# daniel05155/Reinforcement-Learning-in-Music-Generation

Measured on AMD Instinct MI355X. Metric: CW-tokens/sec pretrain fwd+bwd @T=1024, higher is better.
Workload: dtype bf16; 1 GPU; agent_pretrain step (fwd+bwd+clip+Adam), repo dims 512/12/8/2048, synthetic CW tokens (B=512/GPU, T=1024, 7 fields -> 6); per_gpu_batch=512, global_batch=512, seq_len=1024, parallelism=dp1, params=38982227, gemm_table=True

## Files before the change

reinforcement-learning-in-music-generation_amd/csrc/cwlt_common.h:

```cpp
#pragma once
#include <hip/hip_runtime.h>
#include <stdint.h>

#define CWLT_OK 0
#define CWLT_ERR_ARG 1001
#define CWLT_ERR_DTYPE 1002

#define CWLT_F32 0
#define CWLT_BF16 1

typedef float f32x16 __attribute__((ext_vector_type(16)));
typedef float f32x4 __attribute__((ext_vector_type(4)));
typedef uint16_t bf16_t;

namespace cwlt {

constexpr int WAVE = 64;

typedef unsigned int u32x4_t __attribute__((ext_vector_type(4)));
__device__ __forceinline__ __amdgpu_buffer_rsrc_t make_rsrc(const void* base, uint32_t bytes) {
    return __builtin_amdgcn_make_buffer_rsrc(const_cast<void*>(base), (short)0, (int)bytes, 0x00020000);
}
__device__ __forceinline__ uint4 buf_load16(__amdgpu_buffer_rsrc_t r, uint32_t byte_off) {
    const u32x4_t v = __builtin_amdgcn_raw_buffer_load_b128(r, (int)byte_off, 0, 0);
    return make_uint4(v[0], v[1], v[2], v[3]);
}

#define CWLT_U4Z make_uint4(0u, 0u, 0u, 0u)

__device__ __forceinline__ float bf16_to_f32(bf16_t x) { return __uint_as_float(((uint32_t)x) << 16); }

typedef __bf16 hwbf16x2 __attribute__((ext_vector_type(2)));
__device__ __forceinline__ bf16_t f32_to_bf16(float f) { return __builtin_bit_cast(bf16_t, (__bf16)f); }
__device__ __forceinline__ uint32_t f32x2_to_bf16x2(float lo, float hi) {
    hwbf16x2 v;
    v[0] = (__bf16)lo;
    v[1] = (__bf16)hi;
    return __builtin_bit_cast(uint32_t, v);
}

__device__ __forceinline__ float4 load4(const float* p) { return *reinterpret_cast<const float4*>(p); }
__device__ __forceinline__ float4 load4(const bf16_t* p) {
    uint2 r = *reinterpret_cast<const uint2*>(p);
    float4 f;
    f.x = __uint_as_float(r.x << 16);
    f.y = __uint_as_float(r.x & 0xffff0000u);
    f.z = __uint_as_float(r.y << 16);
    f.w = __uint_as_float(r.y & 0xffff0000u);
    return f;
}
__device__ __forceinline__ void store4(float* p, float4 f) { *reinterpret_cast<float4*>(p) = f; }
__device__ __forceinline__ void store4(bf16_t* p, float4 f) {
    uint2 r;
    r.x = f32x2_to_bf16x2(f.x, f.y);
    r.y = f32x2_to_bf16x2(f.z, f.w);
    *reinterpret_cast<uint2*>(p) = r;
}
__device__ __forceinline__ float load1(const float* p) { return *p; }
__device__ __forceinline__ float load1(const bf16_t* p) { return bf16_to_f32(*p); }
__device__ __forceinline__ void store1(float* p, float f) { *p = f; }
__device__ __forceinline__ void store1(bf16_t* p, float f) { *p = f32_to_bf16(f); }

__device__ __forceinline__ void load8(const float* p, float (&x)[8]) {
    float4 a = load4(p), b = load4(p + 4);
    x[0] = a.x; x[1] = a.y; x[2] = a.z; x[3] = a.w; x[4] = b.x; x[5] = b.y; x[6] = b.z; x[7] = b.w;
}
__device__ __forceinline__ void load8(const bf16_t* p, float (&x)[8]) {
    uint4 r = *reinterpret_cast<const uint4*>(p);
    x[0] = __uint_as_float(r.x << 16); x[1] = __uint_as_float(r.x & 0xffff0000u);
    x[2] = __uint_as_float(r.y << 16); x[3] = __uint_as_float(r.y & 0xffff0000u);
    x[4] = __uint_as_float(r.z << 16); x[5] = __uint_as_float(r.z & 0xffff0000u);
    x[6] = __uint_as_float(r.w << 16); x[7] = __uint_as_float(r.w & 0xffff0000u);
}
__device__ __forceinline__ void store8(float* p, const float (&x)[8]) {
    store4(p, make_float4(x[0], x[1], x[2], x[3]));
    store4(p + 4, make_float4(x[4], x[5], x[6], x[7]));
}
__device__ __forceinline__ void store8(bf16_t* p, const float (&x)[8]) {
    uint4 r;
    r.x = f32x2_to_bf16x2(x[0], x[1]);
    r.y = f32x2_to_bf16x2(x[2], x[3]);
    r.z = f32x2_to_bf16x2(x[4], x[5]);
    r.w = f32x2_to_bf16x2(x[6], x[7]);
    *reinterpret_cast<uint4*>(p) = r;
}

template <typename T> struct VecIO;
template <> struct VecIO<float> {
    static constexpr int N = 4;
    static __device__ __forceinline__ void load(const float* p, float (&x)[4]) {
        const float4 a = load4(p);
        x[0] = a.x; x[1] = a.y; x[2] = a.z; x[3] = a.w;
    }
    static __device__ __forceinline__ void store(float* p, const float (&x)[4]) {
        store4(p, make_float4(x[0], x[1], x[2], x[3]));
    }
};
template <> struct VecIO<bf16_t> {
    static constexpr int N = 8;
    static __device__ __forceinline__ void load(const bf16_t* p, float (&x)[8]) { load8(p, x); }
    static __device__ __forceinline__ void store(bf16_t* p, const float (&x)[8]) { store8(p, x); }
};
template <int N>
__device__ __forceinline__ void loadf(const float* p, float (&x)[N]) {
#pragma unroll
    for (int i = 0; i < N; i += 4) {
        const float4 a = load4(p + i);
        x[i] = a.x; x[i + 1] = a.y; x[i + 2] = a.z; x[i + 3] = a.w;
    }
}

template <int CTRL>
__device__ __forceinline__ float dpp_move(float v) {
    return __builtin_bit_cast(float, __builtin_amdgcn_update_dpp(0, __builtin_bit_cast(int, v), CTRL, 0xf, 0xf, false));
}
__device__ __forceinline__ float lane_value(float v, int lane) {
    return __builtin_bit_cast(float, __builtin_amdgcn_readlane(__builtin_bit_cast(int, v), lane));
}
__device__ __forceinline__ float wave_sum(float v) {
    v += dpp_move<0xB1>(v);
    v += dpp_move<0x4E>(v);
    v += dpp_move<0x141>(v);
    v += dpp_move<0x140>(v);
    return (lane_value(v, 0) + lane_value(v, 16)) + (lane_value(v, 32) + lane_value(v, 48));
}
__device__ __forceinline__ float wave_max(float v) {
    v = fmaxf(v, dpp_move<0xB1>(v));
    v = fmaxf(v, dpp_move<0x4E>(v));
    v = fmaxf(v, dpp_move<0x141>(v));
    v = fmaxf(v, dpp_move<0x140>(v));
    return fmaxf(fmaxf(lane_value(v, 0), lane_value(v, 16)), fmaxf(lane_value(v, 32), lane_value(v, 48)));
}

__device__ __forceinline__ uint32_t hash32(uint32_t x) {
    x ^= x >> 16; x *= 0x7feb352du; x ^= x >> 15; x *= 0x846ca68bu; x ^= x >> 16;
    return x;
}
__device__ __forceinline__ uint32_t rng_pair(uint64_t seed, uint64_t pair_idx) {
    const uint32_t lo = (uint32_t)pair_idx, hi = (uint32_t)(pair_idx >> 32);
    const uint32_t key = (uint32_t)seed ^ ((uint32_t)(seed >> 32) * 0x9e3779b9u) ^ (hi * 0x85ebca6bu);
    return hash32(lo * 0x9e3779b1u ^ key);
}
template <int N>
__device__ __forceinline__ uint32_t dropout_mask(uint64_t seed, uint64_t off, uint32_t thresh16) {
    uint32_t m = 0;
#pragma unroll
    for (int j = 0; j < N; j += 2) {
        const uint32_t r = rng_pair(seed, (off >> 1) + (j >> 1));
        m |= ((r & 0xffffu) >= thresh16 ? 1u : 0u) << j;
        m |= ((r >> 16) >= thresh16 ? 1u : 0u) << (j + 1);
    }
    return m;
}
__device__ __forceinline__ bool dropout_keep(uint64_t seed, uint64_t idx, uint32_t thresh16) {
    const uint32_t r = rng_pair(seed, idx >> 1);
    return ((idx & 1) ? (r >> 16) : (r & 0xffffu)) >= thresh16;
}
__device__ __forceinline__ uint32_t keep_lanes16(uint32_t r, uint32_t thresh2) {
    uint32_t m;
    const uint32_t one = 0x00010001u;
    asm("v_pk_sub_u16 %0, %1, %2 clamp\n\t"
        "v_pk_min_u16 %0, %0, %3\n\t"
        "v_pk_sub_u16 %0, %0, %3"
        : "=&v"(m)
        : "s"(thresh2), "v"(r), "s"(one));
    return m;
}

static inline uint32_t drop_thresh(float p) {
    if (p <= 0.f) return 0u;
    long t = (long)((double)p * 65536.0 + 0.5);
    if (t < 1) t = 1;
    if (t > 65535) t = 65535;
    return (uint32_t)t;
}
static inline float drop_scale(float p) {
    const uint32_t t = drop_thresh(p);
    return t ? (float)(65536.0 / (65536.0 - (double)t)) : 1.0f;
}
int launch_colsum_finalize(const float* part, float* out, int nblocks, long stride, int ncols, float scale,
                           int accumulate, hipStream_t st);
int launch_colsum_finalize_multi(const float* part, float* out, long out_stride, int nq, int nblocks, long stride,
                                 int ncols, hipStream_t st);


int launch_gemm_ffn_big(int gelu, const void* a, const void* w, const float* bias, void* g, void* c, float* part,
                        int64_t M, int N, int K, int64_t lda, int64_t ldw, uint32_t thresh, float keep_scale,
                        uint64_t seed, const uint64_t* seed_base, hipStream_t st);
long gemm_ffn_big_tiles(long M);

int scan_segments(int N, int H, int L);
long scan_seg_floats(int N, int H, int P, int backward);
long scan_final_state_floats(int N, int H);
int launch_cla_fwd_bf16(const void* q, const void* k, const void* v, void* out, float* zinv, int N, int H, int L,
                        long ldq, long ldk, long ldv, long ldo, float eps, int P, float* ws, float* fin,
                        hipStream_t st);
int launch_cla_bwd_sweep_bf16(const void* q, const void* k, const void* v, const void* out, const float* zinv,
                              const void* dout, const float* fin, void* dq, void* dk, void* dv, float* csum_q,
                              float* csum_k, float* csum_v, int N, int H, int L, long ldq, long ldk, long ldv, long ldo,
                              long lddo, long lddq, long lddk, long lddv, hipStream_t st);
int launch_cla_bwd_dq_bf16(const void* q, const void* k, const void* v, const void* out, const float* zinv,
                           const void* dout, const float* dden, void* dq, float* csum, int N, int H, int L, long ldq,
                           long ldk, long ldv, long ldo, long lddo, long lddq, int P, float* ws, hipStream_t st);
int launch_cla_bwd_dkdv_bf16(const void* q, const void* k, const void* v, const void* out, const float* zinv,
                             const void* dout, void* dk, void* dv, float* csum_k, float* csum_v, float* dden_out,
                             int N, int H, int L, long ldq, long ldk, long ldv, long ldo, long lddo, long lddk,
                             long lddv, int P, float* ws, hipStream_t st);

}
```

reinforcement-learning-in-music-generation_amd/csrc/gemm_ln.hip:

```cpp
#include "cwlt_common.h"
#include "cwlt_lds_dma.h"
#include <stdlib.h>

namespace cwlt {
namespace gl {

constexpr int TMR = 128, TNC = 512, BK = 32;
constexpr int NSTAGE = 3;
constexpr int STG = (TMR + TNC) * BK * 2;
constexpr int LDE = TNC + 8;
constexpr int LDS_BYTES = TMR * LDE * 2 > NSTAGE * STG ? TMR * LDE * 2 : NSTAGE * STG;

typedef __bf16 bf16x4 __attribute__((ext_vector_type(4)));

__global__ __launch_bounds__(1024) void gemm_ln_kernel(
    const bf16_t* __restrict__ A, const bf16_t* __restrict__ W, const float* __restrict__ bias,
    const bf16_t* __restrict__ X, const float* __restrict__ gamma, const float* __restrict__ beta,
    bf16_t* __restrict__ S, bf16_t* __restrict__ Y, float* __restrict__ mean, float* __restrict__ rstd, long M, int K,
    long lda, long ldw, float eps, uint32_t thresh, float keep_scale, uint64_t seed,
    const uint64_t* __restrict__ seed_base) {
    extern __shared__ __attribute__((aligned(16))) char lds[];

    const int tid = threadIdx.x, lane = tid & 63;
    const int w = __builtin_amdgcn_readfirstlane(tid >> 6);
    const int wm = w >> 3, wn = w & 7;
    const int l31 = lane & 31, hf = lane >> 5;
    const long m0 = (long)blockIdx.x * TMR;
    const long mrows = min((long)TMR, M - m0);

    const uint64_t abase = (uint64_t)(A + m0 * lda), wbase = (uint64_t)W;
    u32x4_t ars, wrs;
    ars[0] = __builtin_amdgcn_readfirstlane((uint32_t)abase);
    ars[1] = __builtin_amdgcn_readfirstlane((uint32_t)(abase >> 32));
    ars[2] = __builtin_amdgcn_readfirstlane((uint32_t)(((mrows - 1) * lda + K) * 2));
    ars[3] = 0x00020000u;
    wrs[0] = __builtin_amdgcn_readfirstlane((uint32_t)wbase);
    wrs[1] = __builtin_amdgcn_readfirstlane((uint32_t)(wbase >> 32));
    wrs[2] = __builtin_amdgcn_readfirstlane((uint32_t)(((long)(TNC - 1) * ldw + K) * 2));
    wrs[3] = 0x00020000u;
    const int dchunk = (lane & 3) ^ ((lane >> 4) & 3);
    const uint32_t a_voff = ((uint32_t)(16 * (w & 7) + (lane >> 2)) * (uint32_t)lda + dchunk * 8) * 2;
    const uint32_t w_voff = ((uint32_t)(32 * w + (lane >> 2)) * (uint32_t)ldw + dchunk * 8) * 2;
    const uint32_t w_16 = (uint32_t)(16 * ldw * 2);
    const uint32_t lds_a = (uint32_t)(uintptr_t)(lds_void*)lds + (w & 7) * 1024;
    const uint32_t lds_w = (uint32_t)(uintptr_t)(lds_void*)lds + TMR * 64 + w * 2048;
#define GL_DMA_W(stage, step)                                                                                     \
    {                                                                                                             \
        unsigned keep;                                                                                            \
        const uint32_t lw = lds_w + (uint32_t)(stage) * STG;                                                      \
        const uint32_t sk_ = (uint32_t)(step) * (BK * 2), sk2 = sk_ + w_16;                                       \
        asm volatile("s_mov_b32 %0, m0\n\ts_mov_b32 m0, %2\n\ts_nop 4\n\t"                                     \
                     "buffer_load_dwordx4 %1, %3, %4 offen lds\n\t"                                               \
                     "s_add_u32 m0, %2, 0x400\n\ts_nop 0\n\t"                                                    \
                     "buffer_load_dwordx4 %1, %3, %5 offen lds\n\t"                                               \
                     "s_mov_b32 m0, %0"                                                                           \
                     : "=&s"(keep)                                                                                \
                     : "v"(w_voff), "s"(lw), "s"(wrs), "s"(sk_), "s"(sk2)                                         \
                     : "memory", "scc");                                                                          \
    }
#define GL_DMA_A(stage, step) lds_dma_piece(a_voff, ars, lds_a + (uint32_t)(stage) * STG, (uint32_t)(step) * (BK * 2))
#define GL_DMA(stage, step)        \
    {                              \
        if (w < 8) GL_DMA_A(stage, step); \
        GL_DMA_W(stage, step);     \
    }
    const int swz = (l31 >> 2) & 3;
    const int of0 = l31 * 64 + ((hf ^ swz) << 4), of1 = l31 * 64 + (((2 + hf) ^ swz) << 4);
    const int oa = (64 * wm) * 64, ow = TMR * 64 + (64 * wn) * 64;
#define GL_FRAG(p) __builtin_bit_cast(bf16x8, *reinterpret_cast<const uint4*>(p))
#define GL_READ(F, stage, ofh)                                            \
    {                                                                     \
        const char* sb = lds + (stage) * STG;                             \
        F[0] = GL_FRAG(sb + ow + (ofh));                                  \
        F[1] = GL_FRAG(sb + ow + 2048 + (ofh));                           \
        F[2] = GL_FRAG(sb + oa + (ofh));                                  \
        F[3] = GL_FRAG(sb + oa + 2048 + (ofh));                           \
    }
#define GL_MFMA(F)                                                                          \
    {                                                                                       \
        acc[0][0] = __builtin_amdgcn_mfma_f32_32x32x16_bf16(F[0], F[2], acc[0][0], 0, 0, 0); \
        acc[0][1] = __builtin_amdgcn_mfma_f32_32x32x16_bf16(F[1], F[2], acc[0][1], 0, 0, 0); \
        acc[1][0] = __builtin_amdgcn_mfma_f32_32x32x16_bf16(F[0], F[3], acc[1][0], 0, 0, 0); \
        acc[1][1] = __builtin_amdgcn_mfma_f32_32x32x16_bf16(F[1], F[3], acc[1][1], 0, 0, 0); \
    }

    f32x16 acc[2][2];
#pragma unroll
    for (int i = 0; i < 2; ++i)
#pragma unroll
        for (int j = 0; j < 2; ++j)
#pragma unroll
            for (int r = 0; r < 16; ++r) acc[i][j][r] = 0.f;

    const int nstep = K / BK;
    bf16x8 F0[4], F1[4];
    GL_DMA(0, 0);
    GL_DMA(1, 1);
    if (nstep > 2) GL_DMA(2, 2);
    if (nstep > 2) {
        if (w < 8)
            asm volatile("s_waitcnt vmcnt(6)" ::: "memory");
        else
            asm volatile("s_waitcnt vmcnt(4)" ::: "memory");
    } else {
        if (w < 8)
            asm volatile("s_waitcnt vmcnt(3)" ::: "memory");
        else
            asm volatile("s_waitcnt vmcnt(2)" ::: "memory");
    }
    __builtin_amdgcn_s_barrier();
    GL_READ(F0, 0, of0);
    int st = 0;
    for (int s = 0; s < nstep; ++s) {
        const int st1 = st == NSTAGE - 1 ? 0 : st + 1;
        GL_READ(F1, st, of1);
        __builtin_amdgcn_sched_barrier(0);
        GL_MFMA(F0);
        __builtin_amdgcn_sched_barrier(0);
        if (s + 1 < nstep) {
            if (s + 2 < nstep) {
                if (w < 8)
                    asm volatile("s_waitcnt vmcnt(3) lgkmcnt(0)" ::: "memory");
                else
                    asm volatile("s_waitcnt vmcnt(2) lgkmcnt(0)" ::: "memory");
            } else {
                asm volatile("s_waitcnt vmcnt(0) lgkmcnt(0)" ::: "memory");
            }
            __builtin_amdgcn_s_barrier();
            __builtin_amdgcn_sched_barrier(0);
            if (s + 3 < nstep) GL_DMA(st, s + 3);
            GL_READ(F0, st1, of0);
            __builtin_amdgcn_sched_barrier(0);
        }
        GL_MFMA(F1);
        __builtin_amdgcn_sched_barrier(0);
        st = st1;
    }
#undef GL_DMA
#undef GL_DMA_A
#undef GL_DMA_W
#undef GL_FRAG
#undef GL_READ
#undef GL_MFMA

    __syncthreads();
    bf16_t* et = reinterpret_cast<bf16_t*>(lds);
#pragma unroll
    for (int i = 0; i < 2; ++i)
#pragma unroll
        for (int j = 0; j < 2; ++j) {
            const int row = 64 * wm + 32 * i + l31, c0 = 64 * wn + 32 * j;
#pragma unroll
            for (int g = 0; g < 4; ++g) {
                bf16x4 p;
#pragma unroll
                for (int u = 0; u < 4; ++u) p[u] = (__bf16)acc[i][j][4 * g + u];
                *reinterpret_cast<uint2*>(et + row * LDE + c0 + 8 * g + 4 * hf) = __builtin_bit_cast(uint2, p);
            }
        }
    const int ecol = lane * 8;
    uint4 xr[8];
    {
        const __amdgpu_buffer_rsrc_t xrs =
            make_rsrc(X + m0 * TNC, (uint32_t)(mrows * TNC * 2));
#pragma unroll
        for (int i = 0; i < 8; ++i) xr[i] = buf_load16(xrs, ((uint32_t)(w + 16 * i) * TNC + ecol) * 2);
    }
    float gm[8], bt[8], bs[8];
    loadf<8>(gamma + ecol, gm);
    loadf<8>(beta + ecol, bt);
    loadf<8>(bias + ecol, bs);
    __syncthreads();
    if (seed_base) seed += *seed_base;
    const float invN = 1.0f / (float)TNC;
#pragma unroll
    for (int i = 0; i < 8; ++i) {
        const int row = w + 16 * i;
        if (row >= mrows) break;
        const uint4 hv = *reinterpret_cast<const uint4*>(et + row * LDE + ecol);
        float v[8], r[8];
        load8(reinterpret_cast<const bf16_t*>(&hv), v);
        load8(reinterpret_cast<const bf16_t*>(&xr[i]), r);
        const long off = (m0 + row) * TNC + ecol;
        const uint32_t km = thresh ? dropout_mask<8>(seed, (uint64_t)off, thresh) : 0xffffffffu;
        float sum = 0.f;
#pragma unroll
        for (int j = 0; j < 8; ++j) {
            const float a = v[j] + bs[j];
            v[j] = (((km >> j) & 1u) ? a * keep_scale : 0.f) + r[j];
            sum += v[j];
        }
        store8(S + off, v);
        const float mu = wave_sum(sum) * invN;
        float sq = 0.f;
#pragma unroll
        for (int j = 0; j < 8; ++j) {
            const float d = v[j] - mu;
            sq = fmaf(d, d, sq);
        }
        const float rs = rsqrtf(wave_sum(sq) * invN + eps);
        float o[8];
#pragma unroll
        for (int j = 0; j < 8; ++j) o[j] = (v[j] - mu) * rs * gm[j] + bt[j];
        store8(Y + off, o);
        if (lane == 0) {
            mean[m0 + row] = mu;
            rstd[m0 + row] = rs;
        }
    }
}

}
}

extern "C" {

int cwlt_gemm_nt_bias_dropout_add_layernorm(const void* a, const void* w, const float* bias, const void* x,
                                            const float* gamma, const float* beta, void* s, void* y, float* mean,
                                            float* rstd, int64_t M, int N, int K, int64_t lda, int64_t ldw, float eps,
                                            float p, uint64_t seed, const uint64_t* seed_base, void* stream) {
    using namespace cwlt;
    if (M < 0 || N != gl::TNC || K <= 0 || (K % 64) || p < 0.f || p >= 1.f) return CWLT_ERR_ARG;
    if (M == 0) return CWLT_OK;
    if (!a || !w || !bias || !x || !gamma || !beta || !s || !y || !mean || !rstd) return CWLT_ERR_ARG;
    if (((lda | ldw) & 7) || lda < K || ldw < K) return CWLT_ERR_ARG;
    if (((uintptr_t)a | (uintptr_t)w | (uintptr_t)x | (uintptr_t)s | (uintptr_t)y | (uintptr_t)bias | (uintptr_t)gamma |
         (uintptr_t)beta) & 15)
        return CWLT_ERR_ARG;
    if ((int64_t)gl::TMR * lda * 2 >= (1ll << 31) || (int64_t)gl::TNC * ldw * 2 >= (1ll << 31)) return CWLT_ERR_ARG;
    static unsigned long long lds_set = 0;
    int dev = 0;
    if (hipGetDevice(&dev) != hipSuccess) dev = 0;
    if (dev >= 64 || !((lds_set >> dev) & 1ull)) {
        const int e = (int)hipFuncSetAttribute((const void*)gl::gemm_ln_kernel, hipFuncAttributeMaxDynamicSharedMemorySize,
                                               gl::LDS_BYTES);
        if (e) return e;
        if (dev < 64) lds_set |= 1ull << dev;
    }
    const long mtiles = (M + gl::TMR - 1) / gl::TMR;
    hipLaunchKernelGGL(gl::gemm_ln_kernel, dim3((unsigned)mtiles), dim3(1024), gl::LDS_BYTES, (hipStream_t)stream,
                       (const bf16_t*)a, (const bf16_t*)w, bias, (const bf16_t*)x, gamma, beta, (bf16_t*)s, (bf16_t*)y, mean,
                       rstd, (long)M, K, (long)lda, (long)ldw, eps, drop_thresh(p), drop_scale(p), seed, seed_base);
    return (int)hipGetLastError();
}

}
```

Measured before the change: 3.273 million CW-tokens/s.

## Add persistent 9-slot LDS-DMA ring GEMM+LayerNorm kernel for large M

Adds a new persistent GEMM + bias + dropout + residual + LayerNorm kernel used when M is at least 32768 rows and K is at least 128. It uses BK=64, 512 threads at two blocks per CU, and a 9-slot LDS ring fed by buffer_load...lds DMA, so weight and A pieces for the next k-steps are prefetched while MFMA runs. Blocks loop over M tiles with next-tile descriptors prepared ahead, and a launch stagger spreads start times. The goal is better MFMA utilisation and overlap than the old 1024-thread 3-stage kernel, at the cost of complex hand-scheduled barriers and inline asm that depend on exact wait counts.

```diff
diff --git a/reinforcement-learning-in-music-generation_amd/csrc/cwlt_common.h b/reinforcement-learning-in-music-generation_amd/csrc/cwlt_common.h
--- a/reinforcement-learning-in-music-generation_amd/csrc/cwlt_common.h
+++ b/reinforcement-learning-in-music-generation_amd/csrc/cwlt_common.h
@@ -188,6 +188,10 @@
                         int64_t M, int N, int K, int64_t lda, int64_t ldw, uint32_t thresh, float keep_scale,
                         uint64_t seed, const uint64_t* seed_base, hipStream_t st);
 long gemm_ffn_big_tiles(long M);
+
+int launch_gemm_ln_big(const void* a, const void* w, const float* bias, const void* x, const float* gamma,
+                       const float* beta, void* s, void* y, float* mean, float* rstd, int64_t M, int K, int64_t lda,
+                       int64_t ldw, float eps, float p, uint64_t seed, const uint64_t* seed_base, hipStream_t st);
 
 int scan_segments(int N, int H, int L);
 long scan_seg_floats(int N, int H, int P, int backward);
diff --git a/reinforcement-learning-in-music-generation_amd/csrc/gemm_bf16_ln.hip b/reinforcement-learning-in-music-generation_amd/csrc/gemm_bf16_ln.hip
--- /dev/null
+++ b/reinforcement-learning-in-music-generation_amd/csrc/gemm_bf16_ln.hip
@@ -0,0 +1,362 @@
+#include "cwlt_common.h"
+#include "cwlt_lds_dma.h"
+#include <stdlib.h>
+
+namespace cwlt {
+namespace gr {
+
+constexpr int TM = 128, TN = 512, BK = 64;
+constexpr int PIECE = 128 * BK * 2;
+constexpr int NSLOT = 9;
+constexpr int RING = NSLOT * PIECE;
+constexpr int STRIP = TN * 4;
+constexpr int STATS = TM * 8 * 4;
+constexpr int LDS_BYTES = RING + 3 * STRIP + 2 * STATS;
+
+#define GR_DMA2(v0, v1, rs, la, so)                                                                    \
+    {                                                                                                  \
+        unsigned keep;                                                                                 \
+        asm volatile("s_mov_b32 %0, m0\n\ts_mov_b32 m0, %4\n\ts_nop 4\n\t"                          \
+                     "buffer_load_dwordx4 %1, %3, %5 offen lds\n\t"                                    \
+                     "s_add_u32 m0, %4, 0x400\n\ts_nop 0\n\t"                                         \
+                     "buffer_load_dwordx4 %2, %3, %5 offen lds\n\t"                                    \
+                     "s_mov_b32 m0, %0"                                                                \
+                     : "=&s"(keep)                                                                     \
+                     : "v"(v0), "v"(v1), "s"(rs), "s"(la), "s"(so)                                     \
+                     : "memory", "scc");                                                               \
+    }
+#define GR_FRAG(off) __builtin_bit_cast(bf16x8, *reinterpret_cast<const uint4*>(lds + (off)))
+#define GR_WAIT(n) asm volatile("s_waitcnt vmcnt(%0)" ::"n"(n) : "memory")
+#define GR_WRAP(x) ((x) >= NSLOT ? (x) - NSLOT : (x))
+
+__global__ __launch_bounds__(512, 2) void gemm_bf16_ln_kernel(
+    const bf16_t* __restrict__ A, const bf16_t* __restrict__ W, const float* __restrict__ bias,
+    const bf16_t* __restrict__ X, const float* __restrict__ gamma, const float* __restrict__ beta, bf16_t* S, bf16_t* Y,
+    float* mean, float* rstd, long M, int K, long lda, long ldw, float eps, uint32_t thresh, float keep_scale,
+    uint64_t seed, const uint64_t* __restrict__ seed_base, int ntile, int stagger) {
+    __shared__ __attribute__((aligned(1024))) char lds[LDS_BYTES];
+    float* lds_bias = reinterpret_cast<float*>(lds + RING);
+    float* lds_gamma = lds_bias + TN;
+    float* lds_beta = lds_gamma + TN;
+    float* lds_stat = lds_beta + TN;
+
+    const int tid = threadIdx.x, lane = tid & 63;
+    const int w = __builtin_amdgcn_readfirstlane(tid >> 6);
+    const bool late = w >= 4;
+    const int l15 = lane & 15, kg = lane >> 4;
+    const int nK = K / BK;
+
+    const int lr = lane >> 3, lp = lane & 7;
+    uint32_t a_voff[2], w_voff[2];
+#pragma unroll
+    for (int i = 0; i < 2; ++i) {
+        const int ch = lp ^ (4 * i + (lane >> 4));
+        a_voff[i] = ((uint32_t)(16 * w + 8 * i + lr) * (uint32_t)lda + ch * 8) * 2;
+        w_voff[i] = ((uint32_t)(64 * w + 16 * i + 8 * (lr >> 2) + (lr & 3)) * (uint32_t)ldw + ch * 8) * 2;
+    }
+    const uint32_t lds_w = (uint32_t)(uintptr_t)(lds_void*)lds + w * 2048;
+    const uint32_t ldw2 = (uint32_t)ldw * 2;
+#define GR_ISSUE_A(rs, tk, slot) GR_DMA2(a_voff[0], a_voff[1], rs, lds_w + (uint32_t)(slot) * PIECE, (uint32_t)(tk) * (BK * 2))
+#define GR_ISSUE_W(nb, tk, slot)                                                            \
+    GR_DMA2(w_voff[0], w_voff[1], wrs, lds_w + (uint32_t)(slot) * PIECE,                    \
+            (uint32_t)(tk) * (BK * 2) + (uint32_t)(32 * ((nb) >> 1) + 4 * ((nb) & 1)) * ldw2)
+
+    int a_off[2], w_off[2];
+#pragma unroll
+    for (int k = 0; k < 2; ++k) {
+        a_off[k] = l15 * 128 + (((kg | (4 * k)) ^ (l15 >> 1)) << 4);
+        w_off[k] = a_off[k] + w * 2048;
+    }
+
+    bf16x8 AF[8][2], WF[2];
+    f32x4 acc[4][8];
+
+#define GR_READ_W(so)                                                                      \
+    _Pragma("unroll") for (int k_ = 0; k_ < 2; ++k_) WF[k_] = GR_FRAG((so) + w_off[k_]);
+#define GR_PHASE(nb, wait)                                                                 \
+    if (wait) GR_WAIT(10);                                                                 \
+    __builtin_amdgcn_s_barrier();                                                          \
+    __builtin_amdgcn_sched_barrier(0);                                                     \
+    __builtin_amdgcn_s_setprio(1);                                                         \
+    _Pragma("unroll") for (int k_ = 0; k_ < 2; ++k_)                                       \
+        _Pragma("unroll") for (int mb_ = 0; mb_ < 8; ++mb_)                                \
+            acc[nb][mb_] = __builtin_amdgcn_mfma_f32_16x16x32_bf16(WF[k_], AF[mb_][k_], acc[nb][mb_], 0, 0, 0); \
+    __builtin_amdgcn_s_setprio(0);                                                         \
+    __builtin_amdgcn_sched_barrier(0);                                                     \
+    __builtin_amdgcn_s_barrier();                                                          \
+    __builtin_amdgcn_sched_barrier(0);
+
+    for (int i = tid; i < TN; i += 512) {
+        lds_bias[i] = bias[i];
+        lds_gamma[i] = gamma[i];
+        lds_beta[i] = beta[i];
+    }
+    if (seed_base) seed += *seed_base;
+
+    u32x4_t ars, arsn, wrs;
+#define GR_DESC(d, ix)                                                                                      \
+    {                                                                                                       \
+        const long m0_ = (long)(ix) * TM;                                                                   \
+        const bool ok_ = (ix) < ntile;                                                                      \
+        const long mr_ = min((long)TM, M - m0_);                                                            \
+        const uint64_t ab_ = (uint64_t)(A + (ok_ ? m0_ * lda : 0));                                         \
+        d[0] = __builtin_amdgcn_readfirstlane((uint32_t)ab_);                                               \
+        d[1] = __builtin_amdgcn_readfirstlane((uint32_t)(ab_ >> 32));                                       \
+        d[2] = __builtin_amdgcn_readfirstlane(ok_ ? (uint32_t)(((mr_ - 1) * lda + K) * 2) : 0u);            \
+        d[3] = 0x00020000u;                                                                                 \
+    }
+    {
+        const uint64_t wb_ = (uint64_t)W;
+        wrs[0] = __builtin_amdgcn_readfirstlane((uint32_t)wb_);
+        wrs[1] = __builtin_amdgcn_readfirstlane((uint32_t)(wb_ >> 32));
+        wrs[2] = __builtin_amdgcn_readfirstlane((uint32_t)(((long)(TN - 1) * ldw + K) * 2));
+        wrs[3] = 0x00020000u;
+    }
+
+    if (stagger) {
+        for (int left = (int)(blockIdx.x >> 3) * stagger; left > 0; left -= 64) __builtin_amdgcn_s_sleep(64);
+    }
+    int idx = (int)blockIdx.x;
+    if (idx >= ntile) return;
+    GR_DESC(ars, idx)
+    __syncthreads();
+    GR_ISSUE_A(ars, 0, 0)
+    GR_ISSUE_W(0, 0, 1)
+    GR_ISSUE_W(1, 0, 2)
+    GR_ISSUE_W(2, 0, 3)
+    GR_ISSUE_W(3, 0, 4)
+    GR_ISSUE_A(ars, 1, 5)
+    GR_ISSUE_W(0, 1, 6)
+    GR_WAIT(0);
+    int ra = 0;
+
+    const float invN = 1.0f / (float)TN;
+    while (true) {
+        const long m0 = (long)idx * TM;
+        const int nxt = idx + (int)gridDim.x;
+        GR_DESC(arsn, nxt)
+#pragma unroll
+        for (int i = 0; i < 4; ++i)
+#pragma unroll
+            for (int j = 0; j < 8; ++j) acc[i][j] = f32x4{0.f, 0.f, 0.f, 0.f};
+        __builtin_amdgcn_s_barrier();
+        __builtin_amdgcn_sched_barrier(0);
+        if (late) __builtin_amdgcn_s_barrier();
+        __builtin_amdgcn_sched_barrier(0);
+
+        for (int t = 0; t < nK; ++t) {
+            const int k1 = t + 1 >= nK ? t + 1 - nK : t + 1;
+            const bool n2 = t + 2 >= nK;
+            const int k2 = n2 ? t + 2 - nK : t + 2;
+            u32x4_t ai;
+            ai[0] = n2 ? arsn[0] : ars[0];
+            ai[1] = n2 ? arsn[1] : ars[1];
+            ai[2] = n2 ? arsn[2] : ars[2];
+            ai[3] = 0x00020000u;
+            const int s_w0 = GR_WRAP(ra + 1), s_w1 = GR_WRAP(ra + 2), s_w2 = GR_WRAP(ra + 3), s_w3 = GR_WRAP(ra + 4);
+            const int s_i1 = GR_WRAP(ra + 7), s_i2 = GR_WRAP(ra + 8);
+            const bool wt = t > 0;
+#pragma unroll
+            for (int k_ = 0; k_ < 2; ++k_)
+#pragma unroll
+                for (int mb_ = 0; mb_ < 8; ++mb_) AF[mb_][k_] = GR_FRAG(ra * PIECE + a_off[k_] + mb_ * 2048);
+            GR_READ_W(s_w0 * PIECE)
+            __builtin_amdgcn_sched_barrier(0);
+            GR_ISSUE_W(1, k1, s_i1)
+            GR_PHASE(0, wt)
+            GR_READ_W(s_w1 * PIECE)
+            __builtin_amdgcn_sched_barrier(0);
+            GR_ISSUE_W(2, k1, s_i2)
+            GR_PHASE(1, wt)
+            GR_READ_W(s_w2 * PIECE)
+            __builtin_amdgcn_sched_barrier(0);
+            GR_ISSUE_W(3, k1, ra)
+            GR_PHASE(2, wt)
+            GR_READ_W(s_w3 * PIECE)
+            __builtin_amdgcn_sched_barrier(0);
+            GR_ISSUE_A(ai, k2, s_w0)
+            GR_ISSUE_W(0, k2, s_w1)
+            GR_PHASE(3, wt)
+            ra = GR_WRAP(ra + 5);
+        }
+        if (!late) __builtin_amdgcn_s_barrier();
+        __builtin_amdgcn_sched_barrier(0);
+
+        const long mrows = min((long)TM, M - m0);
+        const __amdgpu_buffer_rsrc_t xrs = make_rsrc(X + m0 * TN, (uint32_t)(mrows * TN * 2));
+        const __amdgpu_buffer_rsrc_t srs = make_rsrc(S + m0 * TN, (uint32_t)(mrows * TN * 2));
+        const __amdgpu_buffer_rsrc_t yrs = make_rsrc(Y + m0 * TN, (uint32_t)(mrows * TN * 2));
+        uint32_t e0 = (uint32_t)l15 * TN + 64 * w + 8 * kg;
+        asm volatile("" : "+v"(e0));
+        const int col0 = (int)(e0 & (TN - 1));
+        uint32_t c_voff[2];
+#pragma unroll
+        for (int q = 0; q < 2; ++q) c_voff[q] = (e0 + 32 * q) * 2;
+        constexpr uint32_t c_step = 16 * TN * 2;
+        u32x4_t xin[8][2];
+#pragma unroll
+        for (int mb = 0; mb < 8; ++mb)
+#pragma unroll
+            for (int q = 0; q < 2; ++q)
+                xin[mb][q] = __builtin_amdgcn_raw_buffer_load_b128(xrs, (int)(c_voff[q] + mb * c_step), 0, 0);
+#pragma unroll
+        for (int mb = 0; mb < 8; mb += 2)
+            asm volatile("s_waitcnt vmcnt(0)"
+                         : "+v"(xin[mb][0]), "+v"(xin[mb][1]), "+v"(xin[mb + 1][0]), "+v"(xin[mb + 1][1])::"memory");
+        __builtin_amdgcn_sched_barrier(0);
+
+        float mu[8], rs[8];
+#pragma unroll
+        for (int mb = 0; mb < 8; ++mb) mu[mb] = 0.f;
+        const uint32_t thresh2 = thresh | (thresh << 16);
+        const uint32_t seed_key = (uint32_t)seed ^ ((uint32_t)(seed >> 32) * 0x9e3779b9u);
+#pragma unroll
+        for (int q = 0; q < 2; ++q) {
+            float bs[8];
+            loadf<8>(lds_bias + col0 + 32 * q, bs);
+#pragma unroll
+            for (int mb = 0; mb < 8; ++mb) {
+                float r[8];
+                load8(reinterpret_cast<const bf16_t*>(&xin[mb][q]), r);
+                const uint64_t pair = (uint64_t)(m0 * TN + (long)(e0 + 16 * mb * TN + 32 * q)) >> 1;
+                const uint32_t base = (uint32_t)pair * 0x9e3779b1u;
+                const uint32_t key = seed_key ^ ((uint32_t)(pair >> 32) * 0x85ebca6bu);
+#pragma unroll
+                for (int c = 0; c < 4; ++c) {
+                    const uint32_t hw = keep_lanes16(hash32((base + (uint32_t)c * 0x9e3779b1u) ^ key), thresh2);
+                    const uint32_t km[2] = {(uint32_t)((int32_t)(hw << 16) >> 16), (uint32_t)((int32_t)hw >> 16)};
+#pragma unroll
+                    for (int h = 0; h < 2; ++h) {
+                        const int j = 2 * c + h;
+                        const float a = (float)(__bf16)acc[2 * q + (j >> 2)][mb][j & 3] + bs[j];
+                        const float v = __uint_as_float(__float_as_uint(a * keep_scale) & km[h]) + r[j];
+                        acc[2 * q + (j >> 2)][mb][j & 3] = v;
+                        mu[mb] += v;
+                    }
+                }
+            }
+        }
+#pragma unroll
+        for (int q = 0; q < 2; ++q)
+#pragma unroll
+            for (int mb = 0; mb < 8; ++mb) {
+                u32x4_t ps;
+#pragma unroll
+                for (int c = 0; c < 4; ++c)
+                    ps[c] = f32x2_to_bf16x2(acc[2 * q + (c >> 1)][mb][(2 * c) & 3], acc[2 * q + (c >> 1)][mb][(2 * c + 1) & 3]);
+                __builtin_amdgcn_raw_buffer_store_b128(ps, srs, (int)(c_voff[q] + mb * c_step), 0, 0);
+            }
+#pragma unroll
+        for (int mb = 0; mb < 8; ++mb) {
+            mu[mb] += __shfl_xor(mu[mb], 16);
+            mu[mb] += __shfl_xor(mu[mb], 32);
+        }
+#define GR_ROWSUM(buf, val)                                                                          \
+        {                                                                                            \
+            float* st_ = lds_stat + (buf) * (TM * 8);                                                \
+            if (kg == 0) {                                                                           \
+                _Pragma("unroll") for (int mb = 0; mb < 8; ++mb) st_[(e0 >> 9) * 8 + 128 * mb + w] = val[mb]; \
+            }                                                                                        \
+            asm volatile("s_waitcnt lgkmcnt(0)" ::: "memory");                                       \
+            __builtin_amdgcn_s_barrier();                                                            \
+            asm volatile("" ::: "memory");                                                           \
+            _Pragma("unroll") for (int mb = 0; mb < 8; ++mb) {                                       \
+                const float4 p0 = *reinterpret_cast<const float4*>(st_ + (e0 >> 9) * 8 + 128 * mb);       \
+                const float4 p1 = *reinterpret_cast<const float4*>(st_ + (e0 >> 9) * 8 + 128 * mb + 4);   \
+                val[mb] = ((((((p0.x + p0.y) + p0.z) + p0.w) + p1.x) + p1.y) + p1.z) + p1.w;         \
+            }                                                                                        \
+        }
+        GR_ROWSUM(0, mu)
+#pragma unroll
+        for (int mb = 0; mb < 8; ++mb) {
+            mu[mb] *= invN;
+            float sq = 0.f;
+#pragma unroll
+            for (int q = 0; q < 2; ++q)
+#pragma unroll
+                for (int j = 0; j < 8; ++j) {
+                    const float d = acc[2 * q + (j >> 2)][mb][j & 3] - mu[mb];
+                    sq = fmaf(d, d, sq);
+                }
+            sq += __shfl_xor(sq, 16);
+            sq += __shfl_xor(sq, 32);
+            rs[mb] = sq;
+        }
+        GR_ROWSUM(1, rs)
+#pragma unroll
+        for (int mb = 0; mb < 8; ++mb) {
+            rs[mb] = rsqrtf(rs[mb] * invN + eps);
+            asm volatile("" : "+v"(mu[mb]));
+        }
+#pragma unroll
+        for (int q = 0; q < 2; ++q) {
+            float gm[8], bt[8];
+            loadf<8>(lds_gamma + col0 + 32 * q, gm);
+            loadf<8>(lds_beta + col0 + 32 * q, bt);
+#pragma unroll
+            for (int mb = 0; mb < 8; ++mb) {
+                u32x4_t py;
+#pragma unroll
+                for (int c = 0; c < 4; ++c) {
+                    const float v0 = acc[2 * q + (c >> 1)][mb][(2 * c) & 3], v1 = acc[2 * q + (c >> 1)][mb][(2 * c + 1) & 3];
+                    const float o0 = (v0 - mu[mb]) * rs[mb] * gm[2 * c] + bt[2 * c];
+                    const float o1 = (v1 - mu[mb]) * rs[mb] * gm[2 * c + 1] + bt[2 * c + 1];
+                    py[c] = f32x2_to_bf16x2(o0, o1);
+                }
+                __builtin_amdgcn_raw_buffer_store_b128(py, yrs, (int)(c_voff[q] + mb * c_step), 0, 0);
+            }
+        }
+        {
+            float mw = mu[0], rw = rs[0];
+#pragma unroll
+            for (int mb = 1; mb < 8; ++mb) {
+                mw = w == mb ? mu[mb] : mw;
+                rw = w == mb ? rs[mb] : rw;
+            }
+            const __amdgpu_buffer_rsrc_t mrs = make_rsrc(mean + m0, (uint32_t)(mrows * 4));
+            const __amdgpu_buffer_rsrc_t rrs = make_rsrc(rstd + m0, (uint32_t)(mrows * 4));
+            const int so = kg == 0 ? (int)(16 * w + (e0 >> 9)) * 4 : 0x7ffffff0;
+            __builtin_amdgcn_raw_buffer_store_b32(__builtin_bit_cast(uint32_t, mw), mrs, so, 0, 0);
+            __builtin_amdgcn_raw_buffer_store_b32(__builtin_bit_cast(uint32_t, rw), rrs, so, 0, 0);
+        }
+        __builtin_amdgcn_sched_barrier(0);
+        if (nxt >= ntile) break;
+        idx = nxt;
+        ars[0] = arsn[0];
+        ars[1] = arsn[1];
+        ars[2] = arsn[2];
+    }
+    GR_WAIT(0);
+#undef GR_ROWSUM
+#undef GR_PHASE
+#undef GR_READ_W
+#undef GR_ISSUE_W
+#undef GR_ISSUE_A
+#undef GR_DESC
+}
+
+}
+
+int launch_gemm_ln_big(const void* a, const void* w, const float* bias, const void* x, const float* gamma,
+                       const float* beta, void* s, void* y, float* mean, float* rstd, int64_t M, int K, int64_t lda,
+                       int64_t ldw, float eps, float p, uint64_t seed, const uint64_t* seed_base, hipStream_t st) {
+    const long ntile = (M + gr::TM - 1) / gr::TM;
+    if (ntile >= (1ll << 30)) return CWLT_ERR_ARG;
+    static int ncu[64];
+    int dev = 0;
+    if (hipGetDevice(&dev) != hipSuccess || dev < 0 || dev >= 64) dev = 0;
+    if (!ncu[dev]) {
+        int n = 0;
+        if (hipDeviceGetAttribute(&n, hipDeviceAttributeMultiprocessorCount, dev) != hipSuccess || n < 8) n = 256;
+        ncu[dev] = n / 8 * 8;
+    }
+    const long grid = ntile < ncu[dev] ? ntile : ncu[dev];
+    const long ngroup = grid / 8 > 0 ? grid / 8 : 1;
+    const int stagger = K <= 1024 ? (int)(4 * ((K / gr::BK) * 3500L + 20000L) / (8 * ngroup * 64)) : 0;
+    hipLaunchKernelGGL(gr::gemm_bf16_ln_kernel, dim3((unsigned)grid), dim3(512), 0, st, (const bf16_t*)a,
+                       (const bf16_t*)w, bias, (const bf16_t*)x, gamma, beta, (bf16_t*)s, (bf16_t*)y, mean, rstd, (long)M,
+                       K, (long)lda, (long)ldw, eps, drop_thresh(p), drop_scale(p), seed, seed_base, (int)ntile, stagger);
+    return (int)hipGetLastError();
+}
+
+}
diff --git a/reinforcement-learning-in-music-generation_amd/csrc/gemm_ln.hip b/reinforcement-learning-in-music-generation_amd/csrc/gemm_ln.hip
--- a/reinforcement-learning-in-music-generation_amd/csrc/gemm_ln.hip
+++ b/reinforcement-learning-in-music-generation_amd/csrc/gemm_ln.hip
@@ -228,6 +228,14 @@
          (uintptr_t)beta) & 15)
         return CWLT_ERR_ARG;
     if ((int64_t)gl::TMR * lda * 2 >= (1ll << 31) || (int64_t)gl::TNC * ldw * 2 >= (1ll << 31)) return CWLT_ERR_ARG;
+    {
+        const char* e = getenv("CWLT_LN_BIG");
+        const char* r = getenv("CWLT_LN_BIG_MIN_ROWS");
+        const long min_rows = r ? atol(r) : 32768L;
+        if (!(e && e[0] == '0') && M >= min_rows && K >= 128)
+            return launch_gemm_ln_big(a, w, bias, x, gamma, beta, s, y, mean, rstd, M, K, lda, ldw, eps, p, seed, seed_base,
+                                      (hipStream_t)stream);
+    }
     static unsigned long long lds_set = 0;
     int dev = 0;
     if (hipGetDevice(&dev) != hipSuccess) dev = 0;
```

Measured after the change: 3.284 million CW-tokens/s, median of 6. About the same (+0.4%).
